# cc-ai/climategan

Hardware: AMD Instinct MI355X
Metric: 640x640 images/sec (G+D step): per-domain sample slots per second of the joint Masker+Painter training step (update_G + update_D), global batch 32 per domain (higher is better)
Workload: dtype bf16

## Files before the change

climategan_amd/csrc/conv_wgrad.hip:

```cpp
#include "cgan_common.h"
#include <type_traits>

namespace {


struct WgradArgs {
  const uint16_t* x;
  const uint16_t* dy;
  float* dw;
  unsigned x_bytes, dy_bytes;
  float* ws;
  float* bpart;
  int n, h_in, w_in, cin, cin_s;
  int cout, cout_s;
  int kh, kw, stride, pad, dil;
  int h_out, w_out, npix;
  int nchunks, ci_blocks, co_blocks, splits, per_xcd;
  int coop, co_pairs, n_pairs;
  int fold, cpt, tpt, tap_slots;
  CGAN_DEV_ONLY(int dbg;)
  int reflect;
  int x_ups;
  CGAN_DEV_ONLY(unsigned long long* ts;)
};
// ... 200 lines not shown
      const bool xv = pv && ci_ok && (unsigned)iy < (unsigned)p.h_in && (unsigned)ix < (unsigned)p.w_in;
      const unsigned row = (unsigned)(c_nh[i] + (MODE == 1 ? (iy >> 1) : iy));
      const unsigned col = (unsigned)(MODE == 1 ? (ix >> 1) : ix);
      const unsigned off = row * row_b + col * cin_b + cch2;
      wg_dma16(rs_x, dst_x + i * PIECE, xv ? off : 0xffffffffu);
      c_pix[i] += step;
      c_dy[i] += step_dy;
      int sx = c_sx[i] + step_sx, sy = c_sy[i] + step_sy, nh = c_nh[i] + step_nh;
      const bool cx = sx >= wrap_x;
      sx = cx ? sx - wrap_x : sx;
      sy = cx ? sy + p.stride : sy;
      const bool cy = sy >= wrap_y;
      sy = cy ? sy - wrap_y : sy;
      nh = cy ? nh + hx : nh;
      c_sx[i] = sx; c_sy[i] = sy; c_nh[i] = nh;
    }
  };

  f32x4 acc[4][4];
#pragma unroll
  for (int a = 0; a < 4; ++a)
#pragma unroll
    for (int b = 0; b < 4; ++b) acc[a][b] = (f32x4){0.f, 0.f, 0.f, 0.f};

  const bool do_bias = p.bpart != nullptr && slot == 0 && cib == 0;
  f32x4 accb[4];
#pragma unroll
  for (int a = 0; a < 4; ++a) accb[a] = (f32x4){0.f, 0.f, 0.f, 0.f};
  int c = split, buf = 0;
  if (c < p.nchunks) issue(0);
  for (; c < p.nchunks; c += p.splits) {
    const int cn = c + p.splits;
    asm volatile("s_waitcnt lgkmcnt(0)" ::: "memory");
    if (cn < p.nchunks) {
      issue(buf ^ 1);
      asm volatile("s_waitcnt vmcnt(8)" ::: "memory");
    } else {
      asm volatile("s_waitcnt vmcnt(0)" ::: "memory");
    }
    const unsigned char* sdy = wl + buf * 2 * SLAB_BYTES;
    const unsigned char* sx = sdy + SLAB_BYTES;
    u32x4 fa[4], fb[4];
#pragma unroll
    for (int a = 0; a < 4; ++a) fa[a] = tr_frag(sdy, a, lane);
#pragma unroll
    for (int b = 0; b < 4; ++b) fb[b] = tr_frag(sx, b, lane);
#pragma unroll
    for (int a = 0; a < 4; ++a)
#pragma unroll
      for (int b = 0; b < 4; ++b) acc[a][b] = mfma16(as_vec8<T>(fa[a]), as_vec8<T>(fb[b]), acc[a][b]);
    if (do_bias) {
#pragma unroll
      for (int a = 0; a < 4; ++a) accb[a] = mfma16(as_vec8<T>(fa[a]), as_vec8<T>(ones_frag<T>()), accb[a]);
    }
    buf ^= 1;
  }
  if (do_bias) store_bias_row(p.bpart + ((size_t)split * 4 + wave) * p.cout_s, accb, 4, co0, p.cout_s, lane);

  asm volatile("s_waitcnt vmcnt(0) lgkmcnt(0)" ::: "memory");
  __syncthreads();
#pragma unroll
  for (int a = 0; a < 4; ++a)
#pragma unroll
    for (int b = 0; b < 4; ++b)
      *reinterpret_cast<f32x4*>(smem + ((wave * 16 + a * 4 + b) * 64 + lane) * 16) = acc[a][b];
  __syncthreads();
  const int j = lane & 15, g = lane >> 4;
  f32x4* wst = nullptr;
  if (p.ws) {
    const int tile = (slot * p.ci_blocks + cib) * p.co_blocks + cob;
    wst = reinterpret_cast<f32x4*>(p.ws) + ((size_t)split * tiles_n + tile) * 1024;
  }
#pragma unroll
  for (int b = 0; b < 4; ++b) {
    const int a = wave;
    f32x4 s = (f32x4){0.f, 0.f, 0.f, 0.f};
#pragma unroll
    for (int w = 0; w < 4; ++w) {
      const f32x4 v = *reinterpret_cast<const f32x4*>(smem + ((w * 16 + a * 4 + b) * 64 + lane) * 16);
      s[0] += v[0]; s[1] += v[1]; s[2] += v[2]; s[3] += v[3];
    }
    if (wst) {
      wst[(a * 4 + b) * 64 + lane] = s;
      continue;
    }
    int tap, ci;
    const bool col_ok = wgrad_column(p.fold, p.cpt, p.tpt, taps_n, p.cin, slot, cib, b * 16 + j, tap, ci);
#pragma unroll
    for (int r = 0; r < 4; ++r) {
      const int co = co0 + a * 16 + 4 * g + r;
      if (co < p.cout && col_ok && !(CGAN_DBG(p) & 1)) atomicAdd(p.dw + ((size_t)co * p.cin + ci) * taps_n + tap, s[r]);
    }
  }
}



template <typename T, int MODE, int CH = 64, bool TS = false, bool BIAS = false, int G = 2>
__global__ __launch_bounds__(64 * G * G, G == 4 ? 1 : (CH == 64 ? 2 : 4)) void conv_wgrad_coop_kernel(WgradArgs p) {
  constexpr int CHUNK2 = CH, SUB2 = (CH / 8) * PIECE, STAGE2 = 2 * G * SUB2;
  constexpr int PPS = CH / 8, PW = PPS / G;
  static_assert(PW >= 1, "a wave stages at least one piece of each operand");
  extern __shared__ __attribute__((aligned(1024))) unsigned char smem[];
  const int lane = threadIdx.x & 63;
  const int wave = __builtin_amdgcn_readfirstlane(threadIdx.x >> 6);
  const int taps_n = p.kh * p.kw;
  int item = (blockIdx.x & 7) * p.per_xcd + (blockIdx.x >> 3);
  if ((int)(blockIdx.x >> 3) >= p.per_xcd || item >= p.co_pairs * p.n_pairs * p.splits) return;
  const int cop = item % p.co_pairs;
  item /= p.co_pairs;
  const int np = item % p.n_pairs;
  const int split = item / p.n_pairs;
  const int cpairs = p.fold ? 1 : (p.ci_blocks + G - 1) / G;
  auto n_tile = [&](int m, int& slot, int& cib) {
    if (p.fold) { slot = np * G + m; cib = 0; return slot < p.tap_slots; }
    slot = np / cpairs;
    cib = (np - slot * cpairs) * G + m;
    return cib < p.ci_blocks;
  };

  const int prow = lane >> 3, qs = (lane & 7) ^ swz(prow), q8 = qs * 8;
  const int mem = wave / G, half = wave % G;
  const unsigned cin_b = (unsigned)p.cin_s * 2u, cout_b = (unsigned)p.cout_s * 2u;
  const int hx = MODE == 1 ? (p.h_in >> 1) : p.h_in, wx = MODE == 1 ? (p.w_in >> 1) : p.w_in;
  const unsigned row_b = (unsigned)wx * cin_b;
  const wg_rsrc_t rs_x = wg_make_rsrc(p.x, p.x_bytes);
  const wg_rsrc_t rs_dy = wg_make_rsrc(p.dy, p.dy_bytes);
  unsigned dy_c = 0x80000000u;
  {
    const int co = (cop * G + mem) * 64 + q8;
    if ((cop * G + mem) < p.co_blocks && co < p.cout_s) dy_c = (unsigned)prow * cout_b + (unsigned)co * 2u;
  }
  int lx, ly;
  unsigned cch2, x_c;
  {
    int slot, cib, ky, kx, cch;
    bool ok = n_tile(mem, slot, cib);
    if (p.fold) {
      const int tl = qs / p.cpt, tap_l = slot * p.tpt + tl;
      ok = ok && tl < p.tpt && tap_l < taps_n;
      const int tcl = ok ? tap_l : 0;
      ky = tcl / p.kw;
      kx = tcl - ky * p.kw;
      cch = (qs - tl * p.cpt) * 8;
    } else {
      ky = slot / p.kw;
      kx = slot - ky * p.kw;
      cch = cib * 64 + q8;
      ok = ok && cch < p.cin_s;
    }
    const int tap_y = ky * p.dil - p.pad, tap_x = kx * p.dil - p.pad;
    const int lxr = prow * p.stride + tap_x;
    ly = tap_y;
    lx = ok ? lxr : -(1 << 20);
    cch2 = (unsigned)cch * 2u;
    x_c = (unsigned)((tap_y * wx + lxr) * (int)cin_b) + cch2;
  }

  int v_sx, v_sy, v_nh;
  {
    const int pix = split * CHUNK2 + (lane & (PPS - 1)) * 8;
    const int r = pix / p.w_out;
    v_sx = (pix - r * p.w_out) * p.stride;
    const int nn = r / p.h_out;
    v_sy = (r - nn * p.h_out) * p.stride;
    v_nh = nn * hx;
  }
  unsigned u_dy = (unsigned)(split * CHUNK2) * cout_b;
  const int step = p.splits * CHUNK2;
  const int step_r = step / p.w_out;
  const int step_sx = (step - step_r * p.w_out) * p.stride;
  const int step_n = step_r / p.h_out;
  const int step_sy = (step_r - step_n * p.h_out) * p.stride;
  const int step_nh = step_n * hx;
  const int wrap_x = p.w_out * p.stride, wrap_y = p.h_out * p.stride;
  const unsigned step_dy = (unsigned)step * cout_b;

  unsigned v_off = 0;
  auto issue_piece = [&](int b, int k) {
    unsigned char* dst = smem + b * STAGE2 + mem * SUB2 + half * (PW * PIECE);
    if (k < PW) {
      const unsigned off = u_dy + (unsigned)((half * PW + k) * 8) * cout_b + dy_c;
      wg_dma16(rs_dy, dst + k * PIECE, off);
      return;
    }
    const int j = k - PW, i = half * PW + j;
    if (j == 0) v_off = (unsigned)((v_nh + v_sy) * wx + v_sx) * cin_b;
    int iy = __builtin_amdgcn_readlane(v_sy, i) + ly, ix = __builtin_amdgcn_readlane(v_sx, i) + lx;
    if (MODE == 2) {
      iy = iy < 0 ? -iy : (iy >= p.h_in ? 2 * p.h_in - 2 - iy : iy);
      ix = ix < 0 ? -ix : (ix >= p.w_in ? 2 * p.w_in - 2 - ix : ix);
    }
    const bool xv = ((unsigned)iy < (unsigned)p.h_in) & ((unsigned)ix < (unsigned)p.w_in);
    unsigned off;
    if (MODE == 1) off = (unsigned)(__builtin_amdgcn_readlane(v_nh, i) + (iy >> 1)) * row_b + (unsigned)(ix >> 1) * cin_b + cch2;
    else if (MODE == 2) off = (unsigned)(__builtin_amdgcn_readlane(v_nh, i) + iy) * row_b + (unsigned)ix * cin_b + cch2;
    else off = (unsigned)__builtin_amdgcn_readlane((int)v_off, i) + x_c;
    wg_dma16(rs_x, dst + G * SUB2 + j * PIECE, xv ? off : 0xffffffffu);
  };
  auto advance = [&]() {
    u_dy += step_dy;
    int sx = v_sx + step_sx, sy = v_sy + step_sy, nh = v_nh + step_nh;
    const bool cx = sx >= wrap_x;
    sx = cx ? sx - wrap_x : sx;
    sy = cx ? sy + p.stride : sy;
    const bool cy = sy >= wrap_y;
    sy = cy ? sy - wrap_y : sy;
    nh = cy ? nh + hx : nh;
    v_sx = sx; v_sy = sy; v_nh = nh;
  };

  const int wc = wave % G, wn = wave / G;
  f32x4 acc[4][4];
#pragma unroll
  for (int a = 0; a < 4; ++a)
#pragma unroll
    for (int b = 0; b < 4; ++b) acc[a][b] = (f32x4){0.f, 0.f, 0.f, 0.f};

  const bool do_bias = BIAS && p.bpart != nullptr && np == 0 && wn == 0;
  f32x4 accb[4];
#pragma unroll
  for (int a = 0; a < 4; ++a) accb[a] = (f32x4){0.f, 0.f, 0.f, 0.f};
  const int nchunks = (p.npix + CHUNK2 - 1) / CHUNK2;
  int c = split, buf = 0;
  unsigned long long t_a = 0, t_b = 0, ts_sum[4] = {0, 0, 0, 0}, t_start = 0;
  if (TS) t_start = __builtin_readcyclecounter();
  if (c < nchunks) {
#pragma unroll
    for (int k = 0; k < 2 * PW; ++k) issue_piece(0, k);
    advance();
  }
  for (; c < nchunks; c += p.splits) {
    if (TS) t_a = __builtin_readcyclecounter();
    asm volatile("s_waitcnt vmcnt(0) lgkmcnt(0)" ::: "memory");
    if (TS) { t_b = __builtin_readcyclecounter(); ts_sum[0] += t_b - t_a; }
    __syncthreads();
    if (TS) { t_a = __builtin_readcyclecounter(); ts_sum[1] += t_a - t_b; }
    if (c + p.splits < nchunks) {
#pragma unroll
      for (int k = 0; k < 2 * PW; ++k) issue_piece(buf ^ 1, k);
      advance();
    }
    if (TS) { t_b = __builtin_readcyclecounter(); ts_sum[2] += t_b - t_a; }
    const unsigned char* sdy = smem + buf * STAGE2 + wc * SUB2;
    const unsigned char* sx = smem + buf * STAGE2 + (G + wn) * SUB2;
#pragma unroll
    for (int ks = 0; ks < CH / 32; ++ks) {
      u32x4 fa[4], fb[4];
#pragma unroll
      for (int a = 0; a < 4; ++a) fa[a] = tr_frag(sdy + ks * 4 * PIECE, a, lane);
#pragma unroll
      for (int b = 0; b < 4; ++b) fb[b] = tr_frag(sx + ks * 4 * PIECE, b, lane);
#pragma unroll
      for (int a = 0; a < 4; ++a)
#pragma unroll
        for (int b = 0; b < 4; ++b) acc[a][b] = mfma16(as_vec8<T>(fa[a]), as_vec8<T>(fb[b]), acc[a][b]);
      if (BIAS && do_bias) {
#pragma unroll
        for (int a = 0; a < 4; ++a) accb[a] = mfma16(as_vec8<T>(fa[a]), as_vec8<T>(ones_frag<T>()), accb[a]);
      }
    }
    buf ^= 1;
    if (TS) { t_a = __builtin_readcyclecounter(); ts_sum[3] += t_a - t_b; }
  }
  if (BIAS && do_bias && cop * G + wc < p.co_blocks)
    store_bias_row(p.bpart + (size_t)split * p.cout_s, accb, 4, (cop * G + wc) * 64, p.cout_s, lane);
  if (TS && CGAN_WTS(p) && lane == 0) {
    unsigned long long* o = CGAN_WTS(p) + ((size_t)blockIdx.x * (G * G) + wave) * 8;
    o[0] = t_start;
    o[1] = __builtin_readcyclecounter();
    for (int i = 0; i < 4; ++i) o[2 + i] = ts_sum[i];
    o[6] = (unsigned long long)((nchunks - split + p.splits - 1) / p.splits);
  }

  const int cob = cop * G + wc;
  int slot_c, cib_c;
  const bool nt_ok = n_tile(wn, slot_c, cib_c);
  if (cob >= p.co_blocks || !nt_ok) return;
  if (p.ws) {
    const int tiles_n = p.tap_slots * p.ci_blocks * p.co_blocks;
    const int tile = (slot_c * p.ci_blocks + cib_c) * p.co_blocks + cob;
    f32x4* wst = reinterpret_cast<f32x4*>(p.ws) + ((size_t)split * tiles_n + tile) * 1024;
#pragma unroll
    for (int a = 0; a < 4; ++a)
#pragma unroll
      for (int b = 0; b < 4; ++b) wst[(a * 4 + b) * 64 + lane] = acc[a][b];
    return;
  }
  const int j = lane & 15, g = lane >> 4;
#pragma unroll
  for (int b = 0; b < 4; ++b) {
    int tap, ci;
    const bool col_ok = wgrad_column(p.fold, p.cpt, p.tpt, taps_n, p.cin, slot_c, cib_c, b * 16 + j, tap, ci);
#pragma unroll
    for (int a = 0; a < 4; ++a)
#pragma unroll
      for (int r = 0; r < 4; ++r) {
        const int co = cob * 64 + a * 16 + 4 * g + r;
        if (co < p.cout && col_ok && !(CGAN_DBG(p) & 1)) atomicAdd(p.dw + ((size_t)co * p.cin + ci) * taps_n + tap, acc[a][b][r]);
      }
  }
}

constexpr int TL_W = 32, TL_H = 4, TL_XP = 40;
constexpr int TL_XH_BYTES = (TL_H + 2) * TL_XP * 128;
constexpr int TL_DY_BYTES = TL_H * TL_W * 128;

__device__ __forceinline__ u32x4 tr_frag_at(const unsigned char* slab, int q0, int tile, int lane) {
  const int i = lane & 15, g = lane >> 4;
  const int k = i >> 2;
  const int chunk = tile * 2 + ((i & 3) >> 1);
  const int qa = q0 + 8 * g + k, qb = qa + 4;
  const unsigned char* a0 = slab + qa * 128 + ((chunk ^ swz(qa & 7)) << 4) + (i & 1) * 8;
  const unsigned char* a1 = slab + qb * 128 + ((chunk ^ swz(qb & 7)) << 4) + (i & 1) * 8;
  s16x4 lo = __builtin_amdgcn_ds_read_tr16_b64_v4i16((__attribute__((address_space(3))) s16x4*)a0);
  s16x4 hi = __builtin_amdgcn_ds_read_tr16_b64_v4i16((__attribute__((address_space(3))) s16x4*)a1);
  u32x4 r;
  r[0] = (uint16_t)lo[0] | ((uint32_t)(uint16_t)lo[1] << 16);
  r[1] = (uint16_t)lo[2] | ((uint32_t)(uint16_t)lo[3] << 16);
  r[2] = (uint16_t)hi[0] | ((uint32_t)(uint16_t)hi[1] << 16);
  r[3] = (uint16_t)hi[2] | ((uint32_t)(uint16_t)hi[3] << 16);
  return r;
}

template <typename T, int NA = 4, bool BIAS = false>
__global__ __launch_bounds__(256, 2) void conv_wgrad_tile3x3_kernel(WgradArgs p) {
  extern __shared__ __attribute__((aligned(1024))) unsigned char smem[];
  unsigned char* xh = smem;
  unsigned char* dyt = smem + TL_XH_BYTES;
  const int lane = threadIdx.x & 63;
  const int wave = __builtin_amdgcn_readfirstlane(threadIdx.x >> 6);
  int item = (blockIdx.x & 7) * p.per_xcd + (blockIdx.x >> 3);
  if ((int)(blockIdx.x >> 3) >= p.per_xcd || item >= p.co_blocks * p.ci_blocks * p.splits) return;
  const int cob = item % p.co_blocks;
  item /= p.co_blocks;
  const int cib = item % p.ci_blocks;
  const int split = item / p.ci_blocks;

  const int prow = lane >> 3, qs = (lane & 7) ^ swz(prow);
  const unsigned cin_b = (unsigned)p.cin_s * 2u, cout_b = (unsigned)p.cout_s * 2u;
  const __amdgpu_buffer_rsrc_t rs_x = __builtin_amdgcn_make_buffer_rsrc(const_cast<uint16_t*>(p.x), 0, p.x_bytes, 0x00020000);
  const __amdgpu_buffer_rsrc_t rs_dy = __builtin_amdgcn_make_buffer_rsrc(const_cast<uint16_t*>(p.dy), 0, p.dy_bytes, 0x00020000);
  const bool ci_ok = cib * 64 + qs * 8 < p.cin_s, co_ok = cob * 64 + qs * 8 < p.cout_s;
  const unsigned x_c = (unsigned)(cib * 64 + qs * 8) * 2u, dy_c = (unsigned)(cob * 64 + qs * 8) * 2u;

  const int tw = p.w_out / TL_W, th = p.h_out / TL_H;
  const int ntiles = p.n * th * tw;

  auto stage = [&](int t) {
    const int tc = t % tw;
    const int r0 = t / tw;
    const int tr = r0 % th, img = r0 / th;
    const int ty0 = tr * TL_H, tx0 = tc * TL_W;
#pragma unroll
    for (int rr = 0; rr < 2; ++rr) {
      const int r = wave + 4 * rr;
      if (r < TL_H + 2) {
        const int iy = ty0 - 1 + r;
        const unsigned row_off = (unsigned)((img * p.h_in + iy) * p.w_in) * cin_b + x_c;
#pragma unroll
        for (int i5 = 0; i5 < 5; ++i5) {
          const int ix = tx0 - 4 + 8 * i5 + prow;
          const bool ok = ci_ok & ((unsigned)iy < (unsigned)p.h_in) & ((unsigned)ix < (unsigned)p.w_in);
          __builtin_amdgcn_raw_ptr_buffer_load_lds(rs_x, (__attribute__((address_space(3))) void*)(xh + (r * TL_XP + 8 * i5) * 128), 16,
                                                   ok ? row_off + (unsigned)ix * cin_b : 0xffffffffu, 0, 0, 0);
        }
      }
    }
    const int j0 = wave < 2 ? wave * 2 : 4 + (wave - 2) * 6, nj = wave < 2 ? 2 : 6;
#pragma unroll
    for (int jj = 0; jj < 6; ++jj) {
      if (jj < nj) {
        const int j = j0 + jj, r = j >> 2, c8 = (j & 3) * 8;
        const unsigned off = (unsigned)((img * p.h_out + ty0 + r) * p.w_out + tx0 + c8 + prow) * cout_b + dy_c;
        __builtin_amdgcn_raw_ptr_buffer_load_lds(rs_dy, (__attribute__((address_space(3))) void*)(dyt + (r * TL_W + c8) * 128), 16,
                                                 co_ok ? off : 0xffffffffu, 0, 0, 0);
      }
    }
  };

  f32x4 acc[NA][9];
#pragma unroll
  for (int a = 0; a < NA; ++a)
#pragma unroll
    for (int i = 0; i < 9; ++i) acc[a][i] = (f32x4){0.f, 0.f, 0.f, 0.f};

  const bool do_bias = BIAS && p.bpart != nullptr && cib == 0 && wave == 0;
  f32x4 accb[4];
#pragma unroll
  for (int a = 0; a < 4; ++a) accb[a] = (f32x4){0.f, 0.f, 0.f, 0.f};
  for (int t = split; t < ntiles; t += p.splits) {
    __syncthreads();
    stage(t);
    asm volatile("s_waitcnt vmcnt(0)" ::: "memory");
    __syncthreads();
#pragma unroll 1
    for (int ty = 0; ty < TL_H; ++ty) {
      u32x4 fa[NA];
#pragma unroll
      for (int a = 0; a < NA; ++a) fa[a] = tr_frag_at(dyt, ty * TL_W, a, lane);
      if (BIAS && do_bias) {
#pragma unroll
        for (int a = 0; a < NA; ++a) accb[a] = mfma16(as_vec8<T>(fa[a]), as_vec8<T>(ones_frag<T>()), accb[a]);
      }
#pragma unroll
      for (int i = 0; i < 9; ++i) {
        const int jn = wave * 9 + i, tap = jn >> 2, grp = jn & 3;
        const int ky = tap / 3, kx = tap - ky * 3;
        const u32x4 fb = tr_frag_at(xh, (ty + ky) * TL_XP + 3 + kx, grp, lane);
#pragma unroll
        for (int a = 0; a < NA; ++a) acc[a][i] = mfma16(as_vec8<T>(fa[a]), as_vec8<T>(fb), acc[a][i]);
      }
    }
  }

  if (BIAS && do_bias) store_bias_row(p.bpart + (size_t)split * p.cout_s, accb, NA, cob * 64, p.cout_s, lane);
  const int tiles_n = 9 * p.ci_blocks * p.co_blocks;
#pragma unroll
  for (int i = 0; i < 9; ++i) {
    const int jn = wave * 9 + i, tap = jn >> 2, grp = jn & 3;
    const int tile = (tap * p.ci_blocks + cib) * p.co_blocks + cob;
    f32x4* wst = reinterpret_cast<f32x4*>(p.ws) + ((size_t)split * tiles_n + tile) * 1024;
#pragma unroll
    for (int a = 0; a < 4; ++a) wst[(a * 4 + grp) * 64 + lane] = a < NA ? acc[a < NA ? a : 0][i] : (f32x4){0.f, 0.f, 0.f, 0.f};
  }
}

template <int KL>
__global__ __launch_bounds__(256) void wgrad_reduce_kernel(const f32x4* __restrict__ ws, float* __restrict__ dw,
                                                           int splits, int taps, int tap_slots, int ci_blocks,
                                                           int co_blocks, int cout, int cin, int fold, int cpt,
                                                           int tpt, int main_blocks, const float* __restrict__ bpart,
                                                           int bias_rows, int cout_s, float* __restrict__ dbias) {
  if ((int)blockIdx.x >= main_blocks) {
    __shared__ float bsum[16][17];
    const int c16 = (int)threadIdx.x & 15, rl = (int)threadIdx.x >> 4;
    const int ch = ((int)blockIdx.x - main_blocks) * 16 + c16;
    float a0 = 0.f, a1 = 0.f, a2 = 0.f, a3 = 0.f;
    if (ch < cout) {
      int r = rl;
      for (; r + 48 < bias_rows; r += 64) {
        a0 += bpart[(size_t)r * cout_s + ch];
        a1 += bpart[(size_t)(r + 16) * cout_s + ch];
        a2 += bpart[(size_t)(r + 32) * cout_s + ch];
        a3 += bpart[(size_t)(r + 48) * cout_s + ch];
      }
      for (; r < bias_rows; r += 16) a0 += bpart[(size_t)r * cout_s + ch];
    }
    bsum[rl][c16] = (a0 + a1) + (a2 + a3);
    __syncthreads();
    if (rl == 0 && ch < cout) {
      float acc = 0.f;
#pragma unroll
      for (int l = 0; l < 16; ++l) acc += bsum[l][c16];
      dbias[ch] += acc;
    }
    return;
  }
  constexpr int EL = 256 / KL;
  __shared__ f32x4 red[KL][EL];
  const int tiles_n = tap_slots * ci_blocks * co_blocks;
  const int el = threadIdx.x % EL, kl = threadIdx.x / EL;
  const int e = blockIdx.x * EL + el;
  f32x4 s = (f32x4){0.f, 0.f, 0.f, 0.f};
  if (e < tiles_n * 1024) {
    const size_t stride = (size_t)tiles_n * 1024;
#pragma unroll 4
    for (int sp = kl; sp < splits; sp += KL) {
      const f32x4 v = ws[(size_t)sp * stride + e];
      s[0] += v[0]; s[1] += v[1]; s[2] += v[2]; s[3] += v[3];
    }
  }
  if (KL > 1) {
    red[kl][el] = s;
    __syncthreads();
    if (kl != 0) return;
#pragma unroll
    for (int l = 1; l < KL; ++l) {
      const f32x4 v = red[l][el];
      s[0] += v[0]; s[1] += v[1]; s[2] += v[2]; s[3] += v[3];
    }
  }
  if (e >= tiles_n * 1024) return;
  int tile = e >> 10;
  const int frag = (e >> 6) & 15, lane = e & 63;
  const int cob = tile % co_blocks;
  tile /= co_blocks;
  const int cib = tile % ci_blocks, slot = tile / ci_blocks;
  int tap, ci;
  if (!wgrad_column(fold, cpt, tpt, taps, cin, slot, cib, (frag & 3) * 16 + (lane & 15), tap, ci)) return;
#pragma unroll
  for (int r = 0; r < 4; ++r) {
    const int co = cob * 64 + (frag >> 2) * 16 + 4 * (lane >> 4) + r;
    if (co >= cout) continue;
    dw[((size_t)co * cin + ci) * taps + tap] += s[r];
  }
}

template <typename T>
__global__ __launch_bounds__(256) void channel_sum_kernel(const uint16_t* __restrict__ x, float* __restrict__ out,
                                                          long npix, int cs, int c, float* __restrict__ part) {
  extern __shared__ __attribute__((aligned(16))) float sm_cs[];
  const int groups = cs / 8;
  const int ppb = blockDim.x / groups;
  const int gi = threadIdx.x % groups, pl = threadIdx.x / groups;
  float s[8] = {0.f, 0.f, 0.f, 0.f, 0.f, 0.f, 0.f, 0.f};
  if (pl < ppb) {
#pragma unroll 4
    for (long pix = (long)blockIdx.x * ppb + pl; pix < npix; pix += (long)gridDim.x * ppb) {
      const u32x4 v = *reinterpret_cast<const u32x4*>(x + pix * cs + gi * 8);
#pragma unroll
      for (int e = 0; e < 4; ++e) {
        float a, b;
        unpack2<T>(v[e], a, b);
        s[2 * e] += a;
        s[2 * e + 1] += b;
      }
    }
#pragma unroll
    for (int e = 0; e < 8; ++e) sm_cs[(pl * groups + gi) * 8 + e] = s[e];
  }
  __syncthreads();
  for (int ch = threadIdx.x; ch < groups * 8; ch += blockDim.x) {
    if (ch >= c) continue;
    float acc = 0.f;
    for (int l = 0; l < ppb; ++l) acc += sm_cs[l * groups * 8 + ch];
    if (part) part[(size_t)blockIdx.x * cs + ch] = acc;
    else atomicAdd(out + ch, acc);
  }
}

CGAN_KNOB(int, g_wgrad_target, 0);
CGAN_KNOB(int, g_wgrad_dbg, 0);
CGAN_KNOB(int, g_wgrad_coop_min_pix, 32768);
CGAN_KNOB(int, g_wgrad_coop_chunk, 0);
CGAN_KNOB(int, g_wgrad_slots, 512);
CGAN_KNOB(int, g_wgrad_tile, 1);
CGAN_KNOB(int, g_wgrad_coop_g, 0);
CGAN_KNOB(int, g_wgrad_bias_fused, 1);
CGAN_KNOB(int, g_wgrad_ws_cost_pct, 100);
CGAN_KNOB(unsigned long long*, g_wgrad_ts, nullptr);
}

#ifdef CGAN_DEV
extern "C" void cgan_debug_set_wgrad_tsbuf(void* p) { g_wgrad_ts = (unsigned long long*)p; }
extern "C" void cgan_debug_set_wgrad_bias_fused(int v) { g_wgrad_bias_fused = v; }
extern "C" void cgan_debug_set_wgrad_ws_cost(int pct) { g_wgrad_ws_cost_pct = pct > 0 ? pct : 100; }
extern "C" void cgan_debug_set_wgrad_tile3x3(int v) { g_wgrad_tile = v; }
extern "C" void cgan_debug_set_wgrad_slots(int v) { g_wgrad_slots = v > 0 ? v : 512; }
extern "C" void cgan_debug_set_wgrad_coop_chunk(int v) { g_wgrad_coop_chunk = (v == 32 || v == 64) ? v : 0; }

extern "C" void cgan_debug_set_wgrad_coop_min_pixels(int v) { g_wgrad_coop_min_pix = v; }
extern "C" void cgan_debug_set_wgrad_coop_g(int v) { g_wgrad_coop_g = (v == 2 || v == 4) ? v : 0; }

extern "C" void cgan_debug_set_wgrad(int target_workgroups, int dbg) {
  g_wgrad_target = target_workgroups;
  g_wgrad_dbg = dbg;
}
#endif

constexpr int BIAS_MAX_BLOCKS = 512;
constexpr int BIAS_MAX_ROWS = 1024;

struct WgradPlan {
  int fold, cpt, tpt, tap_slots, ci_blocks, co_blocks, splits;
  int coop, co_pairs, n_pairs, chunk;
  int g;
  int tile;
  long tiles() const { return (long)tap_slots * ci_blocks * co_blocks; }
};

static WgradPlan wgrad_plan(const CganConvDesc* d, bool have_ws = true) {
  WgradPlan pl;
  const int taps = d->kh * d->kw, cin_s = cgan_cs(d->c_in);
  pl.co_blocks = ceil_div(cgan_cs(d->c_out), 64);
  pl.fold = (cin_s <= 32 && taps > 1 && g_wgrad_dbg != 4) ? 1 : 0;
  pl.cpt = pl.fold ? cin_s / 8 : 8;
  pl.tpt = pl.fold ? 8 / pl.cpt : 1;
  pl.tap_slots = pl.fold ? ceil_div(taps, pl.tpt) : taps;
  pl.ci_blocks = pl.fold ? 1 : ceil_div(cin_s, 64);
  const long npix = (long)d->n * d->h_out * d->w_out;
  pl.g = 2;
  pl.co_pairs = (pl.co_blocks + 1) / 2;
  pl.n_pairs = pl.fold ? (pl.tap_slots + 1) / 2 : pl.tap_slots * ((pl.ci_blocks + 1) / 2);
  pl.coop = ((pl.co_blocks % 2) == 0 && ((pl.fold ? pl.tap_slots : pl.ci_blocks) % 2) == 0 && (d->w_out % 8) == 0 &&
             (g_wgrad_dbg & 8) == 0 && (double)npix * cgan_cs(d->c_out) * 2.0 < 1.9e9 &&
             (npix >= (long)g_wgrad_coop_min_pix || pl.tiles() >= 256))
                ? 1 : 0;
  pl.tile = ((g_wgrad_tile == 2 || (g_wgrad_tile == 1 && !pl.coop)) && have_ws && !pl.fold && d->kh == 3 && d->kw == 3 && d->stride == 1 && d->pad == 1 &&
             d->dilation == 1 && d->pad_mode == CGAN_PAD_ZERO && !d->in_upsample && (d->w_out % TL_W) == 0 &&
             (d->h_out % TL_H) == 0 && (cin_s % 64) == 0 && npix >= 65536 && (g_wgrad_dbg & (8 | 16)) == 0) ? 1 : 0;
  if (pl.tile) {
    pl.coop = 0;
    pl.chunk = TL_W * TL_H;
    const long pairs = (long)pl.co_blocks * pl.ci_blocks, ntiles = npix / (TL_W * TL_H);
    long sp = g_wgrad_target < 0 ? -g_wgrad_target : (long)g_wgrad_slots / pairs;
    if (sp > ntiles) sp = ntiles;
    pl.splits = sp < 1 ? 1 : (int)sp;
    return pl;
  }
  const long tiles = pl.coop ? (long)pl.co_pairs * pl.n_pairs : pl.tiles();
  auto plan_splits = [&](int chunk, long slots, int& nchunks_out) {
    const int nchunks = (int)((npix + chunk - 1) / chunk);
    nchunks_out = nchunks;
    long sp_best = 1;
    if (g_wgrad_target > 0) {
      sp_best = (g_wgrad_target + tiles - 1) / tiles;
    } else if (g_wgrad_target < 0) {
      sp_best = -g_wgrad_target;
    } else {
      const double t_ws = (pl.coop ? 0.024 : 0.008) * (g_wgrad_ws_cost_pct / 100.0);
      double best = 1e30;
      for (int m = 0; m <= 8; ++m) {
        long sp = m == 0 ? 1 : (slots * m) / tiles;
        if (sp < 1) continue;
        if (sp > nchunks) sp = nchunks;
        const long wgs = sp * tiles;
        const double cost = (double)((wgs + slots - 1) / slots) * ((double)((nchunks + sp - 1) / sp) + 2.0) + (double)wgs * t_ws;
        if (cost < best) { best = cost; sp_best = sp; }
      }
    }
    if (sp_best > nchunks) sp_best = nchunks;
    return sp_best < 1 ? 1L : sp_best;
  };
  int nchunks = 0;
  pl.chunk = pl.coop ? 64 : 128;
  if (pl.coop && g_wgrad_coop_g != 2 && (pl.co_blocks % 4) == 0 && ((pl.fold ? pl.tap_slots : pl.ci_blocks) % 4) == 0 &&
      g_wgrad_coop_chunk == 0) {
    const long tiles4 = (long)(pl.co_blocks / 4) * (pl.fold ? pl.tap_slots / 4 : (long)pl.tap_slots * (pl.ci_blocks / 4));
    const int nch = (int)((npix + 63) / 64);
    long sp = g_wgrad_target < 0 ? -g_wgrad_target : (g_wgrad_slots / 2) / tiles4;
    if (sp < 1) sp = 1;
    if (sp > nch) sp = nch;
    if (g_wgrad_coop_g == 4 || (tiles4 <= g_wgrad_slots / 2 && nch / sp >= 8)) {
      pl.g = 4;
      pl.co_pairs = pl.co_blocks / 4;
      pl.n_pairs = pl.fold ? pl.tap_slots / 4 : pl.tap_slots * (pl.ci_blocks / 4);
      pl.chunk = 64;
      pl.splits = (int)sp;
      return pl;
    }
  }
  long splits = plan_splits(pl.chunk, g_wgrad_slots, nchunks);
  if (pl.coop && (g_wgrad_coop_chunk == 32 || (g_wgrad_coop_chunk == 0 && nchunks / splits >= 96))) {
    pl.chunk = 32;
    splits = plan_splits(32, 2 * g_wgrad_slots, nchunks);
  }
  if (splits > nchunks) splits = nchunks;
  pl.splits = splits < 1 ? 1 : (int)splits;
  return pl;
}

extern "C" size_t cgan_conv2d_bwd_weight_workspace_bytes(const CganConvDesc* d) {
  if (!d || d->n <= 0 || d->h_out <= 0 || d->w_out <= 0 || d->c_in <= 0 || d->c_out <= 0 || d->kh <= 0 || d->kw <= 0)
    return 0;
  const WgradPlan pl = wgrad_plan(d);
  return (size_t)pl.tiles() * (size_t)pl.splits * 64 * 64 * sizeof(float) + (size_t)BIAS_MAX_ROWS * cgan_cs(d->c_out) * sizeof(float);
}

extern "C" int cgan_conv2d_nhwc_bwd_weight(const void* x, const void* dy, float* dw_oihw, float* dbias,
                                           const CganConvDesc* d, void* workspace, size_t workspace_bytes,
                                           void* stream) {
  CGAN_REQUIRE(d != nullptr && x && dy && dw_oihw, "conv2d_nhwc_bwd_weight: null pointer");
  CGAN_REQUIRE(d->dtype == CGAN_F16 || d->dtype == CGAN_BF16, "conv2d_nhwc_bwd_weight: bad dtype %d", d->dtype);
  CGAN_REQUIRE(d->pad_mode == CGAN_PAD_ZERO || d->pad_mode == CGAN_PAD_REFLECT, "conv2d_nhwc_bwd_weight: bad pad mode");
  if (d->pad_mode == CGAN_PAD_REFLECT)
    CGAN_REQUIRE(d->pad < d->h_in && d->pad < d->w_in && !d->in_upsample,
                 "conv2d_nhwc_bwd_weight: reflect padding must be < input size (and is not combined with in_upsample)");
  if (d->in_upsample) CGAN_REQUIRE((d->h_in % 2) == 0 && (d->w_in % 2) == 0, "conv2d_nhwc_bwd_weight: in_upsample needs even h_in/w_in");
  CGAN_REQUIRE(d->n > 0 && d->h_in > 0 && d->w_in > 0 && d->c_in > 0 && d->c_out > 0 && d->kh > 0 && d->kw > 0 &&
                   d->stride > 0 && d->dilation > 0 && d->pad >= 0,
               "conv2d_nhwc_bwd_weight: bad shape");
  const int eh = (d->h_in + 2 * d->pad - d->dilation * (d->kh - 1) - 1) / d->stride + 1;
  const int ew = (d->w_in + 2 * d->pad - d->dilation * (d->kw - 1) - 1) / d->stride + 1;
  CGAN_REQUIRE(eh == d->h_out && ew == d->w_out, "conv2d_nhwc_bwd_weight: h_out/w_out inconsistent");
  WgradArgs a;
  a.x = (const uint16_t*)x; a.dy = (const uint16_t*)dy; a.dw = dw_oihw;
  a.n = d->n; a.h_in = d->h_in; a.w_in = d->w_in; a.cin = d->c_in; a.cin_s = cgan_cs(d->c_in);
  a.cout = d->c_out; a.cout_s = cgan_cs(d->c_out);
  a.kh = d->kh; a.kw = d->kw; a.stride = d->stride; a.pad = d->pad; a.dil = d->dilation;
  a.h_out = d->h_out; a.w_out = d->w_out;
  const long npix = (long)d->n * d->h_out * d->w_out;
  CGAN_REQUIRE(npix < (1L << 31) - 256, "conv2d_nhwc_bwd_weight: too many pixels");
  a.npix = (int)npix;
  a.x_ups = d->in_upsample;
  a.reflect = d->pad_mode == CGAN_PAD_REFLECT;
  a.nchunks = ceil_div(a.npix, 128);
  const WgradPlan pl = wgrad_plan(d, workspace != nullptr);
  a.ci_blocks = pl.ci_blocks; a.co_blocks = pl.co_blocks; a.splits = pl.splits;
  a.fold = pl.fold; a.cpt = pl.cpt; a.tpt = pl.tpt; a.tap_slots = pl.tap_slots;
  a.coop = pl.coop; a.co_pairs = pl.co_pairs; a.n_pairs = pl.n_pairs;
  const int taps = d->kh * d->kw;
  CGAN_DEV_ONLY(a.dbg = g_wgrad_dbg; a.ts = g_wgrad_ts;)
  const long items = (long)a.splits * (pl.tile ? (long)pl.co_blocks * pl.ci_blocks
                                              : (pl.coop ? (long)pl.co_pairs * pl.n_pairs : pl.tiles()));
  a.per_xcd = (int)((items + 7) / 8);
  CGAN_REQUIRE(items < (1L << 30), "conv2d_nhwc_bwd_weight: grid too large");
  const unsigned gx = (unsigned)a.per_xcd * 8;
  a.ws = nullptr;
  a.bpart = nullptr;
  int bias_rows = 0;
  if (workspace) {
    CGAN_REQUIRE(workspace_bytes >= cgan_conv2d_bwd_weight_workspace_bytes(d),
                 "conv2d_nhwc_bwd_weight: workspace too small (%zu bytes)", workspace_bytes);
    a.ws = (float*)workspace;
    const int rows = a.splits * ((pl.tile || pl.coop) ? 1 : 4);
    const bool variant_ok = pl.tile ? (pl.co_blocks == 1 && ceil_div(cgan_cs(d->c_out), 16) < 4)
                                    : (!pl.coop || (pl.chunk == 64 && pl.g == 2));
    if (dbias && rows <= BIAS_MAX_ROWS && variant_ok && g_wgrad_bias_fused && CGAN_WTS(a) == nullptr) {
      a.bpart = a.ws + (size_t)pl.tiles() * (size_t)pl.splits * 64 * 64;
      bias_rows = rows;
    }
  }
  hipStream_t s = (hipStream_t)stream;
  const size_t smem = 4 * WAVE_LDS;
  CGAN_REQUIRE((double)d->n * (a.x_ups ? d->h_in / 2 : d->h_in) * (a.x_ups ? d->w_in / 2 : d->w_in) * a.cin_s * 2.0 < 4294967295.0 &&
                   (double)a.npix * a.cout_s * 2.0 < 4294967295.0,
               "conv2d_nhwc_bwd_weight: activation tensors of 4 GiB or more are not supported");
  a.x_bytes = (unsigned)((size_t)d->n * (a.x_ups ? d->h_in / 2 : d->h_in) * (a.x_ups ? d->w_in / 2 : d->w_in) * a.cin_s * 2);
  a.dy_bytes = (unsigned)((size_t)a.npix * a.cout_s * 2);
  const int mode = a.x_ups ? 1 : (a.reflect ? 2 : 0);
  const bool uni = (d->w_out % 8) == 0 && g_wgrad_dbg != 16 &&
                   ((double)a.npix + (double)a.splits * 128.0 + 128.0) * a.cout_s * 2.0 < 2147483648.0;
#define CGAN_BIG_LDS(KERNEL)                                                                                           \
  do {                                                                                                                 \
    static unsigned long long done_mask = 0;                                                                           \
    int dev_ = 0;                                                                                                      \
    (void)hipGetDevice(&dev_);                                                                                         \
    if (!((done_mask >> (dev_ & 63)) & 1ull)) {                                                                        \
      hipError_t e_ = hipFuncSetAttribute(reinterpret_cast<const void*>(&KERNEL),                                      \
                                          hipFuncAttributeMaxDynamicSharedMemorySize, 160 * 1024);                     \
      if (e_ != hipSuccess) {                                                                                          \
        cgan_set_error("conv2d_nhwc_bwd_weight: hipFuncSetAttribute failed: %s", hipGetErrorString(e_));               \
        return CGAN_ERR_HIP;                                                                                           \
      }                                                                                                                \
      done_mask |= 1ull << (dev_ & 63);                                                                                \
    }                                                                                                                  \
  } while (0)
#define WGRAD_LAUNCH(TT, MM, UU) do { CGAN_BIG_LDS((conv_wgrad_kernel<TT, MM, UU>)); hipLaunchKernelGGL((conv_wgrad_kernel<TT, MM, UU>), dim3(gx), dim3(256), smem, s, a); } while (0)
#define WGRAD_MODE(TT)                                                          \
  do {                                                                          \
    if (mode == 2) { if (uni) WGRAD_LAUNCH(TT, 2, true); else WGRAD_LAUNCH(TT, 2, false); }     \
    else if (mode == 1) { if (uni) WGRAD_LAUNCH(TT, 1, true); else WGRAD_LAUNCH(TT, 1, false); } \
    else { if (uni) WGRAD_LAUNCH(TT, 0, true); else WGRAD_LAUNCH(TT, 0, false); }                \
  } while (0)
  if (pl.tile) {
    const size_t smem3 = TL_XH_BYTES + TL_DY_BYTES;
    const int na = pl.co_blocks == 1 ? ceil_div(a.cout_s, 16) : 4;
#define TILE_LAUNCH(TT, NN, BB) hipLaunchKernelGGL((conv_wgrad_tile3x3_kernel<TT, NN, BB>), dim3(gx), dim3(256), smem3, s, a)
#define TILE_NB(TT, NN) do { if (a.bpart) TILE_LAUNCH(TT, NN, true); else TILE_LAUNCH(TT, NN, false); } while (0)
#define TILE_NA(TT) do { if (na == 1) TILE_NB(TT, 1); else if (na == 2) TILE_NB(TT, 2); else if (na == 3) TILE_NB(TT, 3); else TILE_LAUNCH(TT, 4, false); } while (0)
    if (d->dtype == CGAN_F16) TILE_NA(F16); else TILE_NA(BF16);
#undef TILE_NA
#undef TILE_NB
#undef TILE_LAUNCH
  } else if (pl.coop && pl.g == 4) {
    const size_t smem4 = (size_t)2 * 8 * 8 * PIECE;
#define COOP4_LAUNCH(TT, MM)                                                                                           \
  do {                                                                                                                 \
    CGAN_BIG_LDS((conv_wgrad_coop_kernel<TT, MM, 64, false, false, 4>));                                               \
    hipLaunchKernelGGL((conv_wgrad_coop_kernel<TT, MM, 64, false, false, 4>), dim3(gx), dim3(1024), smem4, s, a);      \
  } while (0)
#define COOP4_MODE(TT) do { if (mode == 1) COOP4_LAUNCH(TT, 1); else if (mode == 2) COOP4_LAUNCH(TT, 2); else COOP4_LAUNCH(TT, 0); } while (0)
#ifdef CGAN_DEV
    if (CGAN_WTS(a) && d->dtype == CGAN_BF16 && mode == 0) {
      CGAN_BIG_LDS((conv_wgrad_coop_kernel<BF16, 0, 64, true, false, 4>));
      hipLaunchKernelGGL((conv_wgrad_coop_kernel<BF16, 0, 64, true, false, 4>), dim3(gx), dim3(1024), smem4, s, a);
    } else
#endif
    if (d->dtype == CGAN_F16) COOP4_MODE(F16);
    else COOP4_MODE(BF16);
#undef COOP4_MODE
#undef COOP4_LAUNCH
  } else if (pl.coop) {
    const size_t smem2 = (size_t)2 * 4 * (pl.chunk / 8) * PIECE;
#define COOP_LAUNCH(TT, MM, CC, BB) do { CGAN_BIG_LDS((conv_wgrad_coop_kernel<TT, MM, CC, false, BB>)); hipLaunchKernelGGL((conv_wgrad_coop_kernel<TT, MM, CC, false, BB>), dim3(gx), dim3(256), smem2, s, a); } while (0)
#define COOP_MODE(TT)                                                                       \
  do {                                                                                      \
    if (pl.chunk == 32) { if (mode == 1) COOP_LAUNCH(TT, 1, 32, false); else if (mode == 2) COOP_LAUNCH(TT, 2, 32, false); else COOP_LAUNCH(TT, 0, 32, false); } \
    else if (a.bpart) { if (mode == 1) COOP_LAUNCH(TT, 1, 64, true); else if (mode == 2) COOP_LAUNCH(TT, 2, 64, true); else COOP_LAUNCH(TT, 0, 64, true); }            \
    else { if (mode == 1) COOP_LAUNCH(TT, 1, 64, false); else if (mode == 2) COOP_LAUNCH(TT, 2, 64, false); else COOP_LAUNCH(TT, 0, 64, false); }            \
  } while (0)
#ifdef CGAN_DEV
    if (CGAN_WTS(a) && d->dtype == CGAN_BF16 && mode == 0) {
      if (pl.chunk == 32) hipLaunchKernelGGL((conv_wgrad_coop_kernel<BF16, 0, 32, true>), dim3(gx), dim3(256), smem2, s, a);
      else { CGAN_BIG_LDS((conv_wgrad_coop_kernel<BF16, 0, 64, true>)); hipLaunchKernelGGL((conv_wgrad_coop_kernel<BF16, 0, 64, true>), dim3(gx), dim3(256), smem2, s, a); }
    } else
#endif
    if (d->dtype == CGAN_F16) COOP_MODE(F16);
    else COOP_MODE(BF16);
#undef COOP_MODE
#undef COOP_LAUNCH
  } else if (d->dtype == CGAN_F16) WGRAD_MODE(F16); else WGRAD_MODE(BF16);
#undef WGRAD_MODE
#undef WGRAD_LAUNCH
  CGAN_CHECK_LAUNCH("conv2d_nhwc_bwd_weight");
  float* bpart = a.bpart;
  if (dbias && !a.bpart) {
    const int cs = a.cout_s;
    const int threads = 256;
    const int ppb = threads / (cs / 8) > 0 ? threads / (cs / 8) : 1;
    CGAN_REQUIRE(cs / 8 <= threads, "conv2d_nhwc_bwd_weight: too many channels for the bias reduction");
    long want = (npix + (long)ppb * 16 - 1) / ((long)ppb * 16);
    const int grid = (int)(want < 1 ? 1 : (want > BIAS_MAX_BLOCKS ? BIAS_MAX_BLOCKS : want));
    const size_t smem_b = (size_t)ppb * (cs / 8) * 8 * sizeof(float);
    if (a.ws) {
      bpart = a.ws + (size_t)pl.tiles() * (size_t)pl.splits * 64 * 64;
      bias_rows = grid;
    }
    if (d->dtype == CGAN_F16)
      hipLaunchKernelGGL(channel_sum_kernel<F16>, dim3(grid), dim3(threads), smem_b, s, (const uint16_t*)dy, dbias, npix,
                         cs, d->c_out, bpart);
    else
      hipLaunchKernelGGL(channel_sum_kernel<BF16>, dim3(grid), dim3(threads), smem_b, s, (const uint16_t*)dy, dbias, npix,
                         cs, d->c_out, bpart);
    CGAN_CHECK_LAUNCH("conv2d_nhwc_bwd_weight(bias)");
  }
  if (a.ws) {
    const int elems = (int)pl.tiles() * 1024;
    const int bias_blocks = bpart ? ceil_div(d->c_out, 16) : 0;
    if (a.splits <= 4) {
      const int mb = ceil_div(elems, 256);
      hipLaunchKernelGGL(wgrad_reduce_kernel<1>, dim3(mb + bias_blocks), dim3(256), 0, s, (const f32x4*)a.ws, a.dw,
                         a.splits, taps, a.tap_slots, a.ci_blocks, a.co_blocks, a.cout, a.cin, a.fold, a.cpt, a.tpt, mb,
                         (const float*)bpart, bias_rows, a.cout_s, dbias);
    } else {
      const int mb = ceil_div(elems, 32);
      hipLaunchKernelGGL(wgrad_reduce_kernel<8>, dim3(mb + bias_blocks), dim3(256), 0, s, (const f32x4*)a.ws, a.dw,
                         a.splits, taps, a.tap_slots, a.ci_blocks, a.co_blocks, a.cout, a.cin, a.fold, a.cpt, a.tpt, mb,
                         (const float*)bpart, bias_rows, a.cout_s, dbias);
    }
    CGAN_CHECK_LAUNCH("conv2d_nhwc_bwd_weight(reduce)");
  }
  return CGAN_OK;
}
```

Baseline: 56.74.

## Generalize tiled 3x3 wgrad kernel to dilated convs and 16-wide tiles

Extends the LDS-tiled 3x3 weight-gradient kernel to handle dilation 2 and 4 and a 16x8 tile shape in addition to 32x4. A host-side geometry picker chooses the tile width that minimizes halo pixels within an LDS budget. The selection heuristic also changes: the tile path is now chosen only when there are enough pixel tiles per split. Dilated convolutions, such as ASPP-style layers, can then avoid the generic or cooperative wgrad paths. In exchange, the kernel uses runtime halo sizes and loops that are no longer fully unrolled, and LDS use can grow.

```diff
diff --git a/climategan_amd/csrc/conv_wgrad.hip b/climategan_amd/csrc/conv_wgrad.hip
--- a/climategan_amd/csrc/conv_wgrad.hip
+++ b/climategan_amd/csrc/conv_wgrad.hip
@@ -526,15 +526,16 @@
   }
 }
 
-constexpr int TL_W = 32, TL_H = 4, TL_XP = 40;
-constexpr int TL_XH_BYTES = (TL_H + 2) * TL_XP * 128;
-constexpr int TL_DY_BYTES = TL_H * TL_W * 128;
-
-__device__ __forceinline__ u32x4 tr_frag_at(const unsigned char* slab, int q0, int tile, int lane) {
-  const int i = lane & 15, g = lane >> 4;
-  const int k = i >> 2;
+constexpr int TL_PIX = 128;
+constexpr int TL_DY_BYTES = TL_PIX * 128;
+constexpr int TL_MAX_LDS = 80 * 1024;
+constexpr int tl_xp(int tw, int d) { return (tw + 2 * d + 7) & ~7; }
+constexpr int tl_halo_px(int tw, int d) { return (TL_PIX / tw + 2 * d) * tl_xp(tw, d); }
+
+__device__ __forceinline__ u32x4 tr_frag_q(const unsigned char* slab, int qa, int tile, int lane) {
+  const int i = lane & 15;
   const int chunk = tile * 2 + ((i & 3) >> 1);
-  const int qa = q0 + 8 * g + k, qb = qa + 4;
+  const int qb = qa + 4;
   const unsigned char* a0 = slab + qa * 128 + ((chunk ^ swz(qa & 7)) << 4) + (i & 1) * 8;
   const unsigned char* a1 = slab + qb * 128 + ((chunk ^ swz(qb & 7)) << 4) + (i & 1) * 8;
   s16x4 lo = __builtin_amdgcn_ds_read_tr16_b64_v4i16((__attribute__((address_space(3))) s16x4*)a0);
@@ -546,12 +547,17 @@
   r[3] = (uint16_t)hi[2] | ((uint32_t)(uint16_t)hi[3] << 16);
   return r;
 }
-
-template <typename T, int NA = 4, bool BIAS = false>
+__device__ __forceinline__ u32x4 tr_frag_at(const unsigned char* slab, int q0, int tile, int lane) {
+  return tr_frag_q(slab, q0 + 8 * (lane >> 4) + ((lane & 15) >> 2), tile, lane);
+}
+
+template <typename T, int NA = 4, bool BIAS = false, int TW = 32>
 __global__ __launch_bounds__(256, 2) void conv_wgrad_tile3x3_kernel(WgradArgs p) {
+  constexpr int TH = TL_PIX / TW;
   extern __shared__ __attribute__((aligned(1024))) unsigned char smem[];
+  const int D = p.dil, XP = tl_xp(TW, D), XR = TH + 2 * D, ppr = XP >> 3;
   unsigned char* xh = smem;
-  unsigned char* dyt = smem + TL_XH_BYTES;
+  unsigned char* dyt = smem + XR * XP * 128;
   const int lane = threadIdx.x & 63;
   const int wave = __builtin_amdgcn_readfirstlane(threadIdx.x >> 6);
   int item = (blockIdx.x & 7) * p.per_xcd + (blockIdx.x >> 3);
@@ -568,38 +574,40 @@
   const bool ci_ok = cib * 64 + qs * 8 < p.cin_s, co_ok = cob * 64 + qs * 8 < p.cout_s;
   const unsigned x_c = (unsigned)(cib * 64 + qs * 8) * 2u, dy_c = (unsigned)(cob * 64 + qs * 8) * 2u;
 
-  const int tw = p.w_out / TL_W, th = p.h_out / TL_H;
+  const int tw = p.w_out / TW, th = p.h_out / TH;
   const int ntiles = p.n * th * tw;
 
+  int dy_j0 = 0, dy_nj = 0;
+  {
+    const int quota = (XR * ppr + 16 + 3) >> 2;
+    int left = 16;
+    for (int w = 0; w < 4; ++w) {
+      const int want = quota - ((XR - w + 3) >> 2) * ppr;
+      const int n = w == 3 ? left : (want < 0 ? 0 : (want > left ? left : want));
+      if (w == wave) { dy_j0 = 16 - left; dy_nj = n; }
+      left -= n;
+    }
+  }
   auto stage = [&](int t) {
     const int tc = t % tw;
     const int r0 = t / tw;
     const int tr = r0 % th, img = r0 / th;
-    const int ty0 = tr * TL_H, tx0 = tc * TL_W;
-#pragma unroll
-    for (int rr = 0; rr < 2; ++rr) {
-      const int r = wave + 4 * rr;
-      if (r < TL_H + 2) {
-        const int iy = ty0 - 1 + r;
-        const unsigned row_off = (unsigned)((img * p.h_in + iy) * p.w_in) * cin_b + x_c;
-#pragma unroll
-        for (int i5 = 0; i5 < 5; ++i5) {
-          const int ix = tx0 - 4 + 8 * i5 + prow;
-          const bool ok = ci_ok & ((unsigned)iy < (unsigned)p.h_in) & ((unsigned)ix < (unsigned)p.w_in);
-          __builtin_amdgcn_raw_ptr_buffer_load_lds(rs_x, (__attribute__((address_space(3))) void*)(xh + (r * TL_XP + 8 * i5) * 128), 16,
-                                                   ok ? row_off + (unsigned)ix * cin_b : 0xffffffffu, 0, 0, 0);
-        }
+    const int ty0 = tr * TH, tx0 = tc * TW;
+    for (int r = wave; r < XR; r += 4) {
+      const int iy = ty0 - D + r;
+      const unsigned row_off = (unsigned)((img * p.h_in + iy) * p.w_in) * cin_b + x_c;
+      for (int i = 0; i < ppr; ++i) {
+        const int ix = tx0 - D + 8 * i + prow;
+        const bool ok = ci_ok & ((unsigned)iy < (unsigned)p.h_in) & ((unsigned)ix < (unsigned)p.w_in);
+        __builtin_amdgcn_raw_ptr_buffer_load_lds(rs_x, (__attribute__((address_space(3))) void*)(xh + (r * XP + 8 * i) * 128), 16,
+                                                 ok ? row_off + (unsigned)ix * cin_b : 0xffffffffu, 0, 0, 0);
       }
     }
-    const int j0 = wave < 2 ? wave * 2 : 4 + (wave - 2) * 6, nj = wave < 2 ? 2 : 6;
-#pragma unroll
-    for (int jj = 0; jj < 6; ++jj) {
-      if (jj < nj) {
-        const int j = j0 + jj, r = j >> 2, c8 = (j & 3) * 8;
-        const unsigned off = (unsigned)((img * p.h_out + ty0 + r) * p.w_out + tx0 + c8 + prow) * cout_b + dy_c;
-        __builtin_amdgcn_raw_ptr_buffer_load_lds(rs_dy, (__attribute__((address_space(3))) void*)(dyt + (r * TL_W + c8) * 128), 16,
-                                                 co_ok ? off : 0xffffffffu, 0, 0, 0);
-      }
+    for (int jj = 0; jj < dy_nj; ++jj) {
+      const int j = dy_j0 + jj, r = (j * 8) / TW, c8 = (j * 8) % TW;
+      const unsigned off = (unsigned)((img * p.h_out + ty0 + r) * p.w_out + tx0 + c8 + prow) * cout_b + dy_c;
+      __builtin_amdgcn_raw_ptr_buffer_load_lds(rs_dy, (__attribute__((address_space(3))) void*)(dyt + j * 8 * 128), 16,
+                                               co_ok ? off : 0xffffffffu, 0, 0, 0);
     }
   };
 
@@ -613,16 +621,17 @@
   f32x4 accb[4];
 #pragma unroll
   for (int a = 0; a < 4; ++a) accb[a] = (f32x4){0.f, 0.f, 0.f, 0.f};
+  const int lane_q = ((8 * (lane >> 4)) / TW) * XP + (8 * (lane >> 4)) % TW + ((lane & 15) >> 2);
   for (int t = split; t < ntiles; t += p.splits) {
     __syncthreads();
     stage(t);
     asm volatile("s_waitcnt vmcnt(0)" ::: "memory");
     __syncthreads();
 #pragma unroll 1
-    for (int ty = 0; ty < TL_H; ++ty) {
+    for (int c = 0; c < TL_PIX / 32; ++c) {
       u32x4 fa[NA];
 #pragma unroll
-      for (int a = 0; a < NA; ++a) fa[a] = tr_frag_at(dyt, ty * TL_W, a, lane);
+      for (int a = 0; a < NA; ++a) fa[a] = tr_frag_at(dyt, c * 32, a, lane);
       if (BIAS && do_bias) {
 #pragma unroll
         for (int a = 0; a < NA; ++a) accb[a] = mfma16(as_vec8<T>(fa[a]), as_vec8<T>(ones_frag<T>()), accb[a]);
@@ -631,7 +640,7 @@
       for (int i = 0; i < 9; ++i) {
         const int jn = wave * 9 + i, tap = jn >> 2, grp = jn & 3;
         const int ky = tap / 3, kx = tap - ky * 3;
-        const u32x4 fb = tr_frag_at(xh, (ty + ky) * TL_XP + 3 + kx, grp, lane);
+        const u32x4 fb = tr_frag_q(xh, (c * (32 / TW) + ky * D) * XP + kx * D + lane_q, grp, lane);
 #pragma unroll
         for (int a = 0; a < NA; ++a) acc[a][i] = mfma16(as_vec8<T>(fa[a]), as_vec8<T>(fb), acc[a][i]);
       }
@@ -771,6 +780,9 @@
 extern "C" void cgan_debug_set_wgrad_bias_fused(int v) { g_wgrad_bias_fused = v; }
 extern "C" void cgan_debug_set_wgrad_ws_cost(int pct) { g_wgrad_ws_cost_pct = pct > 0 ? pct : 100; }
 extern "C" void cgan_debug_set_wgrad_tile3x3(int v) { g_wgrad_tile = v; }
+static int g_wgrad_last_kernel = 0, g_wgrad_last_splits = 0;
+extern "C" int cgan_debug_wgrad_last_kernel(void) { return g_wgrad_last_kernel; }
+extern "C" int cgan_debug_wgrad_last_splits(void) { return g_wgrad_last_splits; }
 extern "C" void cgan_debug_set_wgrad_slots(int v) { g_wgrad_slots = v > 0 ? v : 512; }
 extern "C" void cgan_debug_set_wgrad_coop_chunk(int v) { g_wgrad_coop_chunk = (v == 32 || v == 64) ? v : 0; }
 
@@ -793,6 +805,16 @@
   int tile;
   long tiles() const { return (long)tap_slots * ci_blocks * co_blocks; }
 };
+
+static int tl_geometry(int h_out, int w_out, int dil) {
+  int best = 0, best_px = 0;
+  for (int tw = 32; tw >= 16; tw /= 2) {
+    const int px = tl_halo_px(tw, dil);
+    if ((w_out % tw) != 0 || (h_out % (TL_PIX / tw)) != 0 || px * 128 + TL_DY_BYTES > TL_MAX_LDS) continue;
+    if (!best || px < best_px) { best = tw; best_px = px; }
+  }
+  return best;
+}
 
 static WgradPlan wgrad_plan(const CganConvDesc* d, bool have_ws = true) {
   WgradPlan pl;
@@ -811,16 +833,21 @@
              (g_wgrad_dbg & 8) == 0 && (double)npix * cgan_cs(d->c_out) * 2.0 < 1.9e9 &&
              (npix >= (long)g_wgrad_coop_min_pix || pl.tiles() >= 256))
                 ? 1 : 0;
-  pl.tile = ((g_wgrad_tile == 2 || (g_wgrad_tile == 1 && !pl.coop)) && have_ws && !pl.fold && d->kh == 3 && d->kw == 3 && d->stride == 1 && d->pad == 1 &&
-             d->dilation == 1 && d->pad_mode == CGAN_PAD_ZERO && !d->in_upsample && (d->w_out % TL_W) == 0 &&
-             (d->h_out % TL_H) == 0 && (cin_s % 64) == 0 && npix >= 65536 && (g_wgrad_dbg & (8 | 16)) == 0) ? 1 : 0;
+  const int tl_tw = (!pl.fold && d->kh == 3 && d->kw == 3 && d->stride == 1 && d->pad == d->dilation &&
+                     (d->dilation == 1 || d->dilation == 2 || d->dilation == 4) && d->pad_mode == CGAN_PAD_ZERO &&
+                     !d->in_upsample && (cin_s % 64) == 0 && (g_wgrad_dbg & (8 | 16)) == 0)
+                        ? tl_geometry(d->h_out, d->w_out, d->dilation) : 0;
+  const long tl_pairs = (long)pl.co_blocks * pl.ci_blocks, tl_ntiles = npix / TL_PIX;
+  long tl_splits = g_wgrad_target < 0 ? -g_wgrad_target : (long)g_wgrad_slots / tl_pairs;
+  if (tl_splits > tl_ntiles) tl_splits = tl_ntiles;
+  if (tl_splits < 1) tl_splits = 1;
+  const bool tl_wins = !pl.coop && npix >= 65536 && tl_ntiles >= 8 * tl_splits;
+  pl.tile = (have_ws && tl_tw && (g_wgrad_tile == 3 || (g_wgrad_tile == 2 && npix >= 65536) || (g_wgrad_tile == 1 && tl_wins)))
+                ? tl_tw : 0;
   if (pl.tile) {
     pl.coop = 0;
-    pl.chunk = TL_W * TL_H;
-    const long pairs = (long)pl.co_blocks * pl.ci_blocks, ntiles = npix / (TL_W * TL_H);
-    long sp = g_wgrad_target < 0 ? -g_wgrad_target : (long)g_wgrad_slots / pairs;
-    if (sp > ntiles) sp = ntiles;
-    pl.splits = sp < 1 ? 1 : (int)sp;
+    pl.chunk = TL_PIX;
+    pl.splits = (int)tl_splits;
     return pl;
   }
   const long tiles = pl.coop ? (long)pl.co_pairs * pl.n_pairs : pl.tiles();
@@ -969,15 +996,17 @@
     else { if (uni) WGRAD_LAUNCH(TT, 0, true); else WGRAD_LAUNCH(TT, 0, false); }                \
   } while (0)
   if (pl.tile) {
-    const size_t smem3 = TL_XH_BYTES + TL_DY_BYTES;
+    const size_t smem3 = (size_t)tl_halo_px(pl.tile, d->dilation) * 128 + TL_DY_BYTES;
     const int na = pl.co_blocks == 1 ? ceil_div(a.cout_s, 16) : 4;
-#define TILE_LAUNCH(TT, NN, BB) hipLaunchKernelGGL((conv_wgrad_tile3x3_kernel<TT, NN, BB>), dim3(gx), dim3(256), smem3, s, a)
+#define TILE_LAUNCH_W(TT, NN, BB, WW) do { CGAN_BIG_LDS((conv_wgrad_tile3x3_kernel<TT, NN, BB, WW>)); hipLaunchKernelGGL((conv_wgrad_tile3x3_kernel<TT, NN, BB, WW>), dim3(gx), dim3(256), smem3, s, a); } while (0)
+#define TILE_LAUNCH(TT, NN, BB) do { if (pl.tile == 16) TILE_LAUNCH_W(TT, NN, BB, 16); else TILE_LAUNCH_W(TT, NN, BB, 32); } while (0)
 #define TILE_NB(TT, NN) do { if (a.bpart) TILE_LAUNCH(TT, NN, true); else TILE_LAUNCH(TT, NN, false); } while (0)
 #define TILE_NA(TT) do { if (na == 1) TILE_NB(TT, 1); else if (na == 2) TILE_NB(TT, 2); else if (na == 3) TILE_NB(TT, 3); else TILE_LAUNCH(TT, 4, false); } while (0)
     if (d->dtype == CGAN_F16) TILE_NA(F16); else TILE_NA(BF16);
 #undef TILE_NA
 #undef TILE_NB
 #undef TILE_LAUNCH
+#undef TILE_LAUNCH_W
   } else if (pl.coop && pl.g == 4) {
     const size_t smem4 = (size_t)2 * 8 * 8 * PIECE;
 #define COOP4_LAUNCH(TT, MM)                                                                                           \
@@ -1019,6 +1048,7 @@
 #undef WGRAD_MODE
 #undef WGRAD_LAUNCH
   CGAN_CHECK_LAUNCH("conv2d_nhwc_bwd_weight");
+  CGAN_DEV_ONLY(g_wgrad_last_kernel = pl.tile ? (pl.tile == 16 ? 5 : 4) : (pl.coop ? (pl.g == 4 ? 3 : 2) : 1); g_wgrad_last_splits = pl.splits;)
   float* bpart = a.bpart;
   if (dbias && !a.bpart) {
     const int cs = a.cout_s;
```

Result: no change. 56.27 (-0.8%).
